# MCG-NJU/MeMOTR

Measured on AMD Instinct MI355X. Metric: train_frames_per_sec, higher is better.
Workload: dtype f32

## Files before the change

### memotr_amd/csrc/clip_ops.hip

```cpp
#include <hip/hip_runtime.h>
#include <stdint.h>
#include <stdio.h>

#include <atomic>

#include "../../include/clip_ops_hip.h"
#include "assign_core.h"

namespace {

thread_local char g_err[256] = {0};

int fail(int code, const char *msg) {
    snprintf(g_err, sizeof(g_err), "%s", msg);
    return code;
}

int check_launch(const char *what) {
    const hipError_t e = hipGetLastError();
    if (e != hipSuccess) {
        snprintf(g_err, sizeof(g_err), "%s: %s", what, hipGetErrorString(e));
        return (int)e;
    }
    g_err[0] = 0;
    return 0;
}

typedef float f32x4_t __attribute__((ext_vector_type(4)));
typedef double f64x4_t __attribute__((ext_vector_type(4)));

struct Box {
    float x1, y1, x2, y2;
};

__device__ __forceinline__ Box to_xyxy(float cx, float cy, float w, float h) {
#pragma clang fp contract(off)
    Box b;
    b.x1 = cx - 0.5f * w;
    b.y1 = cy - 0.5f * h;
    b.x2 = cx + 0.5f * w;
    b.y2 = cy + 0.5f * h;
    return b;
}

__device__ __forceinline__ float giou_pair(const Box a, const Box b) {
#pragma clang fp contract(off)
    const float iw = fmaxf(fminf(a.x2, b.x2) - fmaxf(a.x1, b.x1), 0.f);
    const float ih = fmaxf(fminf(a.y2, b.y2) - fmaxf(a.y1, b.y1), 0.f);
    const float inter = iw * ih;
    const float area_a = (a.x2 - a.x1) * (a.y2 - a.y1);
    const float area_b = (b.x2 - b.x1) * (b.y2 - b.y1);
    const float uni = area_a + area_b - inter;
    const float iou = inter / uni;
    const float hw = fmaxf(fmaxf(a.x2, b.x2) - fminf(a.x1, b.x1), 0.f);
    const float hh = fmaxf(fmaxf(a.y2, b.y2) - fminf(a.y1, b.y1), 0.f);
    const float hull = hw * hh;
    return iou - (hull - uni) / hull;
}

__device__ __forceinline__ float sigmoidf(float x) { return 1.f / (1.f + expf(-x)); }

__device__ __forceinline__ float powg(float x, float gamma) { return gamma == 2.f ? x * x : powf(x, gamma); }

__global__ __launch_bounds__(256) void match_cost_kernel(const float *__restrict__ logits, long lsl, long lsq,
                                                        const float *__restrict__ boxes, long bsl, long bsq,
                                                        const int64_t *__restrict__ gt_labels,
                                                        const float *__restrict__ gt_boxes, int n_layers, int Q,
                                                        int K, int T, float w_class, float w_bbox, float w_giou,
                                                        float *__restrict__ cost) {
#pragma clang fp contract(off)
    const long total = (long)n_layers * Q * T;
    for (long i = (long)blockIdx.x * blockDim.x + threadIdx.x; i < total; i += (long)gridDim.x * blockDim.x) {
        const int t = (int)(i % T);
        const long lq = i / T;
        const int q = (int)(lq % Q), l = (int)(lq / Q);
        long lab = gt_labels[t];
        lab = lab < 0 ? 0 : (lab >= K ? K - 1 : lab);
        const float prob = sigmoidf(logits[l * lsl + q * lsq + lab]);
        const float alpha = 0.25f, gamma = 2.f;
        const float neg = ((1.f - alpha) * powg(prob, gamma)) * (-logf(1.f - prob + 1e-8f));
        const float pos = (alpha * powg(1.f - prob, gamma)) * (-logf(prob + 1e-8f));
        const float c_class = pos - neg;
        const float *pb = boxes + l * bsl + q * bsq;
        const float *tb = gt_boxes + (long)t * 4;
        const float p0 = pb[0], p1 = pb[1], p2 = pb[2], p3 = pb[3];
        const float t0 = tb[0], t1 = tb[1], t2 = tb[2], t3 = tb[3];
        const float c_bbox = ((fabsf(p0 - t0) + fabsf(p1 - t1)) + fabsf(p2 - t2)) + fabsf(p3 - t3);
        const float giou = giou_pair(to_xyxy(p0, p1, p2, p3), to_xyxy(t0, t1, t2, t3));
        cost[i] = (w_bbox * c_bbox + w_class * c_class) + w_giou * (-giou);
    }
}

__global__ __launch_bounds__(256) void pair_box_loss_fwd_kernel(const float *__restrict__ boxes,
                                                               const int64_t *__restrict__ lay,
                                                               const int64_t *__restrict__ qidx, long row_mul,
                                                               long row_add, const float *__restrict__ tgt,
                                                               const int64_t *__restrict__ gidx,
                                                               const float *__restrict__ weight, int n,
                                                               float *__restrict__ l1, float *__restrict__ gl) {
#pragma clang fp contract(off)
    const int i = blockIdx.x * blockDim.x + threadIdx.x;
    if (i >= n) return;
    const float *pb = boxes + (lay[i] * row_mul + row_add + qidx[i]) * 4;
    const float *tb = tgt + (gidx ? gidx[i] : (long)i) * 4;
    const float p0 = pb[0], p1 = pb[1], p2 = pb[2], p3 = pb[3];
    const float t0 = tb[0], t1 = tb[1], t2 = tb[2], t3 = tb[3];
    float a = ((fabsf(p0 - t0) + fabsf(p1 - t1)) + fabsf(p2 - t2)) + fabsf(p3 - t3);
    float g = 1.f - giou_pair(to_xyxy(p0, p1, p2, p3), to_xyxy(t0, t1, t2, t3));
    if (weight) {
        a *= weight[i];
        g *= weight[i];
    }
    l1[i] = a;
    gl[i] = g;
}

__device__ __forceinline__ float iou_pair(const Box a, const Box b) {
#pragma clang fp contract(off)
    const float iw = fmaxf(fminf(a.x2, b.x2) - fmaxf(a.x1, b.x1), 0.f);
    const float ih = fmaxf(fminf(a.y2, b.y2) - fmaxf(a.y1, b.y1), 0.f);
    const float inter = iw * ih;
    const float uni = (a.x2 - a.x1) * (a.y2 - a.y1) + (b.x2 - b.x1) * (b.y2 - b.y1) - inter;
    return inter / uni;
}

__global__ __launch_bounds__(256) void pair_iou_kernel(const float *__restrict__ boxes, const float *__restrict__ tgt,
                                                      const int64_t *__restrict__ gidx, int n,
                                                      float *__restrict__ iou) {
#pragma clang fp contract(off)
    const int i = blockIdx.x * blockDim.x + threadIdx.x;
    if (i >= n) return;
    const float *pb = boxes + (long)i * 4;
    const float *tb = tgt + (gidx ? gidx[i] : (long)i) * 4;
    iou[i] = iou_pair(to_xyxy(pb[0], pb[1], pb[2], pb[3]), to_xyxy(tb[0], tb[1], tb[2], tb[3]));
}

struct HandoverCols {
    int K, C, QW, oB, oR, oO, oM, oS, oQ, oI, W;
};

HandoverCols handover_cols(int K, int C, int use_dab) {
    HandoverCols c;
    c.K = K;
    c.C = C;
    c.QW = use_dab ? C : 2 * C;
    c.oB = K;
    c.oR = K + 4;
    c.oO = K + 8;
    c.oM = c.oO + C;
    c.oS = c.oM + C;
    c.oQ = c.oS + C;
    c.oI = c.oQ + c.QW;
    c.W = c.oI + 1;
    return c;
}

// ... 933 lines not shown
                        lo = sr_bf16(sr_to_bf16(lo)) + sr_bf16((uint16_t)(rw[k] & 0xffffu));
                        hi = sr_bf16(sr_to_bf16(hi)) + sr_bf16((uint16_t)(rw[k] >> 16));
                    }
                    lo = lo < 0.f ? 0.f : lo;
                    hi = hi < 0.f ? 0.f : hi;
                    vw[k] = (unsigned)sr_to_bf16(lo) | ((unsigned)sr_to_bf16(hi) << 16);
                }
                reinterpret_cast<uint4 *>(xp)[i] = v;
            }
        } else {
            for (long i = (long)blockIdx.x * blockDim.x + threadIdx.x; i < HW; i += (long)gridDim.x * blockDim.x) {
                float v = sr_bf16(xp[i]) + b;
                if (RES) v = sr_bf16(sr_to_bf16(v)) + sr_bf16(rp[i]);
                xp[i] = sr_to_bf16(v < 0.f ? 0.f : v);
            }
        }
    }
}


typedef float lb_f32x16 __attribute__((ext_vector_type(16)));

#ifndef MSDA_LB_U
#define MSDA_LB_U 4
#endif
constexpr int LB_U = MSDA_LB_U;

template <bool GX, bool RELU>
__device__ __forceinline__ void linear_bwd_tile(const float *__restrict__ g, const float *__restrict__ y,
                                                const float *__restrict__ Bp, int M, int N, int K, int OUT, int i0, int j0,
                                                float *__restrict__ C, float *__restrict__ gb, float (*s_c)[16][64],
                                                float (*s_b)[32]) {
    const int lane = threadIdx.x & 63, wave = threadIdx.x >> 6;
    const int i = i0 + (lane & 31), j = j0 + (lane & 31), kq = (lane >> 5) * 4;
    const bool iok = i < M, jok = j < N;
    const int chunks = (K + 7) / 8, per = (chunks + 3) / 4;
    const int c_lo = wave * per, c_hi = (c_lo + per) < chunks ? (c_lo + per) : chunks;
    const bool vec = GX && (OUT % 4 == 0);
    lb_f32x16 acc = {0.f, 0.f, 0.f, 0.f, 0.f, 0.f, 0.f, 0.f, 0.f, 0.f, 0.f, 0.f, 0.f, 0.f, 0.f, 0.f};
    float bsum = 0.f;
    for (int c = c_lo; c < c_hi; c += LB_U) {
        float a[LB_U][4], b[LB_U][4], m[LB_U][4];
#pragma unroll
        for (int u = 0; u < LB_U; ++u) {
            const int k0 = (c + u) * 8 + kq;
            const bool cok = c + u < c_hi;
            if (vec) {
                float4 av = {0.f, 0.f, 0.f, 0.f}, mv = {1.f, 1.f, 1.f, 1.f};
                if (cok && iok && k0 < K) {
                    av = *reinterpret_cast<const float4 *>(g + (long)i * OUT + k0);
                    if (RELU) mv = *reinterpret_cast<const float4 *>(y + (long)i * OUT + k0);
                }
                a[u][0] = av.x; a[u][1] = av.y; a[u][2] = av.z; a[u][3] = av.w;
                m[u][0] = mv.x; m[u][1] = mv.y; m[u][2] = mv.z; m[u][3] = mv.w;
            }
#pragma unroll
            for (int q = 0; q < 4; ++q) {
                const int k = k0 + q;
                const bool kok = cok && k < K;
                if (!vec) {
                    const long idx = GX ? (long)i * OUT + k : (long)k * OUT + i;
                    a[u][q] = (iok && kok) ? g[idx] : 0.f;
                    m[u][q] = (RELU && iok && kok) ? y[idx] : 1.f;
                }
                b[u][q] = (jok && kok) ? Bp[(long)k * N + j] : 0.f;
            }
        }
#pragma unroll
        for (int u = 0; u < LB_U; ++u) {
#pragma unroll
            for (int q = 0; q < 4; ++q) {
                const float av = RELU ? (m[u][q] <= 0.f ? 0.f : a[u][q]) : a[u][q];
                acc = __builtin_amdgcn_mfma_f32_32x32x2f32(av, b[u][q], acc, 0, 0, 0);
                bsum += av;
            }
        }
    }
#pragma unroll
    for (int r = 0; r < 16; ++r) s_c[wave][r][lane] = acc[r];
    bsum += __shfl_xor(bsum, 32, 64);
    if (lane < 32) s_b[wave][lane] = bsum;
    __syncthreads();
#pragma unroll
    for (int rr = 0; rr < 4; ++rr) {
        const int r = wave * 4 + rr;
        const float v = (s_c[0][r][lane] + s_c[1][r][lane]) + (s_c[2][r][lane] + s_c[3][r][lane]);
        const int row = i0 + (r & 3) + 8 * (r >> 2) + 4 * (lane >> 5);
        if (row < M && jok) C[(long)row * N + j] = v;
    }
    if (!GX && gb != nullptr && j0 == 0 && wave == 0 && lane < 32 && i0 + lane < M)
        gb[i0 + lane] = (s_b[0][lane] + s_b[1][lane]) + (s_b[2][lane] + s_b[3][lane]);
}

template <bool RELU>
__global__ __launch_bounds__(256) void linear_bwd_kernel(const float *__restrict__ g, const float *__restrict__ y,
                                                         const float *__restrict__ x, const float *__restrict__ w,
                                                         int R, int IN, int OUT, float *__restrict__ gx,
                                                         float *__restrict__ gw, float *__restrict__ gb, int n_gx,
                                                         int gx_tj, int gw_tj) {
    __shared__ float s_c[4][16][64];
    __shared__ float s_b[4][32];
    const int tile = blockIdx.x;
    if (tile < n_gx) {
        linear_bwd_tile<true, RELU>(g, y, w, R, IN, OUT, OUT, (tile / gx_tj) * 32, (tile % gx_tj) * 32, gx, nullptr, s_c, s_b);
    } else {
        const int t = tile - n_gx;
        linear_bwd_tile<false, RELU>(g, y, x, OUT, IN, R, OUT, (t / gw_tj) * 32, (t % gw_tj) * 32, gw, gb, s_c, s_b);
    }
}

template <bool RELU>
__global__ __launch_bounds__(256) void linear_fwd_kernel(const float *__restrict__ x, const float *__restrict__ w,
                                                         const float *__restrict__ bias, int R, int IN, int OUT,
                                                         float *__restrict__ yout, int tj) {
    __shared__ float s_c[4][16][64];
    const int lane = threadIdx.x & 63, wave = threadIdx.x >> 6;
    const int i0 = (blockIdx.x / tj) * 32, j0 = (blockIdx.x % tj) * 32;
    const int i = i0 + (lane & 31), j = j0 + (lane & 31), kq = (lane >> 5) * 4;
    const bool iok = i < R, jok = j < OUT;
    const int chunks = (IN + 7) / 8, per = (chunks + 3) / 4;
    const int c_lo = wave * per, c_hi = (c_lo + per) < chunks ? (c_lo + per) : chunks;
    lb_f32x16 acc = {0.f, 0.f, 0.f, 0.f, 0.f, 0.f, 0.f, 0.f, 0.f, 0.f, 0.f, 0.f, 0.f, 0.f, 0.f, 0.f};
    for (int c = c_lo; c < c_hi; c += LB_U) {
        float4 a[LB_U], b[LB_U];
#pragma unroll
        for (int u = 0; u < LB_U; ++u) {
            const int k0 = (c + u) * 8 + kq;
            const bool kok = c + u < c_hi && k0 < IN;
            a[u] = (iok && kok) ? *reinterpret_cast<const float4 *>(x + (long)i * IN + k0) : float4{0.f, 0.f, 0.f, 0.f};
            b[u] = (jok && kok) ? *reinterpret_cast<const float4 *>(w + (long)j * IN + k0) : float4{0.f, 0.f, 0.f, 0.f};
        }
#pragma unroll
        for (int u = 0; u < LB_U; ++u) {
            acc = __builtin_amdgcn_mfma_f32_32x32x2f32(a[u].x, b[u].x, acc, 0, 0, 0);
            acc = __builtin_amdgcn_mfma_f32_32x32x2f32(a[u].y, b[u].y, acc, 0, 0, 0);
            acc = __builtin_amdgcn_mfma_f32_32x32x2f32(a[u].z, b[u].z, acc, 0, 0, 0);
            acc = __builtin_amdgcn_mfma_f32_32x32x2f32(a[u].w, b[u].w, acc, 0, 0, 0);
        }
    }
#pragma unroll
    for (int r = 0; r < 16; ++r) s_c[wave][r][lane] = acc[r];
    __syncthreads();
    const float bj = (bias != nullptr && jok) ? bias[j] : 0.f;
#pragma unroll
    for (int rr = 0; rr < 4; ++rr) {
        const int r = wave * 4 + rr;
        float v = ((s_c[0][r][lane] + s_c[1][r][lane]) + (s_c[2][r][lane] + s_c[3][r][lane])) + bj;
        if (RELU) v = v < 0.f ? 0.f : v;
        const int row = i0 + (r & 3) + 8 * (r >> 2) + 4 * (lane >> 5);
        if (row < R && jok) yout[(long)row * OUT + j] = v;
    }
}

}

__global__ __launch_bounds__(256) void track_ownership_kernel(const int64_t *__restrict__ tr_ids, int n_tr,
                                                              const int64_t *__restrict__ gt_ids, int n_gt,
                                                              int64_t *__restrict__ matched, float *__restrict__ free_out) {
    for (int i = threadIdx.x; i < n_tr; i += blockDim.x) {
        const int64_t id = tr_ids[i];
        int64_t m = -1;
        for (int j = 0; j < n_gt; ++j)
            if (gt_ids[j] == id) m = j;
        matched[i] = m;
    }
    for (int j = threadIdx.x; j < n_gt; j += blockDim.x) {
        const int64_t id = gt_ids[j];
        bool owned = false;
        for (int i = 0; i < n_tr; ++i) owned = owned || tr_ids[i] == id;
        free_out[j] = owned ? 0.f : 1.f;
    }
}

__global__ __launch_bounds__(256) void focal_labels_kernel(const int64_t *__restrict__ lay, const int64_t *__restrict__ q,
                                                           const int64_t *__restrict__ g, int n_pairs,
                                                           const int64_t *__restrict__ gt_labels, int n_gt,
                                                           const int64_t *__restrict__ matched, int n_tr,
                                                           const unsigned char *__restrict__ late, int n_layers, int nd,
                                                           int K, int64_t *__restrict__ labels) {
    const int nq = nd + n_tr;
    for (int e = threadIdx.x; e < n_layers * nq; e += blockDim.x) {
        const int l = e / nq, c = e - l * nq;
        int64_t v = K;
        if (c >= nd && late[l]) {
            const int64_t m = matched[c - nd];
            if (m >= 0 && m < n_gt) v = gt_labels[m];
        }
        labels[e] = v;
    }
    __syncthreads();
    for (int p = threadIdx.x; p < n_pairs; p += blockDim.x) {
        const int64_t l = lay[p], c = q[p], t = g[p];
        if (l >= 0 && l < n_layers && c >= 0 && c < nq && t >= 0 && t < n_gt) labels[l * nq + c] = gt_labels[t];
    }
}

__global__ __launch_bounds__(256) void result_rows_kernel(const float *__restrict__ boxes, const float *__restrict__ scores,
                                                          const int64_t *__restrict__ ids,
                                                          const int64_t *__restrict__ labels, int n, int K, int64_t frame,
                                                          float ori_w, float ori_h, float score_thresh, float area_thresh,
                                                          float *__restrict__ rows_f, int64_t *__restrict__ rows_i,
                                                          int32_t *__restrict__ counters, int capacity) {
    __shared__ int wave_total[4];
    const int lane = threadIdx.x & 63, wave = threadIdx.x >> 6;
    const int stored0 = counters[0], dropped0 = counters[1];
    int base = 0;
    for (int c0 = 0; c0 < n; c0 += 256) {
        const int i = c0 + (int)threadIdx.x;
        bool keep = false;
        float s = 0.f, cx = 0.f, cy = 0.f, w = 0.f, h = 0.f;
        if (i < n) {
            const float *sc = scores + (long)i * K;
            s = sc[0];
            for (int k = 1; k < K; ++k) {
                const float v = sc[k];
                if (v > s || v != v) s = v;
            }
            cx = boxes[4 * i], cy = boxes[4 * i + 1], w = boxes[4 * i + 2], h = boxes[4 * i + 3];
            const float area = __fmul_rn(__fmul_rn(__fmul_rn(w, ori_w), h), ori_h);
            keep = s > score_thresh && area > area_thresh;
        }
        const unsigned long long m = __ballot(keep);
        const int below = __popcll(m & ((1ull << lane) - 1ull));
        if (lane == 0) wave_total[wave] = __popcll(m);
        __syncthreads();
        int before = 0, total = 0;
        for (int v = 0; v < 4; ++v) {
            const int t = wave_total[v];
            before += v < wave ? t : 0;
            total += t;
        }
        if (keep) {
            const long pos = (long)stored0 + base + before + below;
            if (pos >= 0 && pos < capacity) {
                const float hw = __fmul_rn(0.5f, w), hh = __fmul_rn(0.5f, h);
                float *rf = rows_f + pos * 5;
                rf[0] = __fmul_rn(__fsub_rn(cx, hw), ori_w);
                rf[1] = __fmul_rn(__fsub_rn(cy, hh), ori_h);
                rf[2] = __fmul_rn(__fadd_rn(cx, hw), ori_w);
                rf[3] = __fmul_rn(__fadd_rn(cy, hh), ori_h);
                rf[4] = s;
                int64_t *ri = rows_i + pos * 3;
                ri[0] = frame;
                ri[1] = ids[i];
                ri[2] = labels[i];
            }
        }
        base += total;
        __syncthreads();
    }
    if (threadIdx.x == 0) {
        const int room = stored0 < 0 ? 0 : (capacity > stored0 ? capacity - stored0 : 0);
        const int stored = base < room ? base : room;
        counters[0] = stored0 + stored;
        counters[1] = dropped0 + (base - stored);
    }
}

template <int NW>
__device__ __forceinline__ void bank_ranks(bool flag, int lane, int wave, int *wave_total, int &before, int &total) {
    const unsigned long long m = __ballot(flag);
    const int below = __popcll(m & ((1ull << lane) - 1ull));
    if (lane == 0) wave_total[wave] = __popcll(m);
    __syncthreads();
    before = below;
    total = 0;
    for (int v = 0; v < NW; ++v) {
        const int t = wave_total[v];
        before += v < wave ? t : 0;
        total += t;
    }
}

constexpr int BANK_THREADS = 1024, BANK_WAVES = BANK_THREADS / 64;

__global__ __launch_bounds__(BANK_THREADS) void bank_update_kernel(clipops_bank_model m, clipops_bank bank, int n_det, int cap,
                                                          int K, int C, int use_dab, float det_thresh,
                                                          float track_thresh, int64_t miss_tolerance) {
#pragma clang fp contract(off)
    __shared__ int wave_total[BANK_WAVES], wave_live[BANK_WAVES], pair_row[BANK_THREADS], pair_slot[BANK_THREADS];
    const int b = blockIdx.x, lane = threadIdx.x & 63, wave = threadIdx.x >> 6;
    const int QW = use_dab ? C : 2 * C;
    const long bc = (long)b * cap;
    int64_t *ids = bank.ids + bc, *labels = bank.labels + bc, *dtime = bank.disappear_time + bc;
    int32_t *free_list = bank.free_list + bc;
    float *boxes = bank.boxes + bc * 4, *ref_pts = bank.ref_pts + bc * 4;
    float *logits = bank.logits + bc * K, *scores = bank.scores + bc * K;
    float *out_embed = bank.output_embed + bc * C, *long_mem = bank.long_memory + bc * C;
    float *last_out = bank.last_output + bc * C, *query = bank.query_embed + bc * QW;
    const float *m_logits = m.ptr[CLIPOPS_BK_LOGITS] + b * m.batch_stride[CLIPOPS_BK_LOGITS];
    const float *m_boxes = m.ptr[CLIPOPS_BK_BOXES] + b * m.batch_stride[CLIPOPS_BK_BOXES];
    const float *m_out = m.ptr[CLIPOPS_BK_OUTPUTS] + b * m.batch_stride[CLIPOPS_BK_OUTPUTS];
    const float *m_ref = m.ptr[CLIPOPS_BK_LAST_REF] + b * m.batch_stride[CLIPOPS_BK_LAST_REF];
    const float *m_query = m.ptr[CLIPOPS_BK_QUERIES] + b * m.batch_stride[CLIPOPS_BK_QUERIES];
    const long rs_logits = m.row_stride[CLIPOPS_BK_LOGITS], rs_boxes = m.row_stride[CLIPOPS_BK_BOXES];
    const long rs_out = m.row_stride[CLIPOPS_BK_OUTPUTS], rs_ref = m.row_stride[CLIPOPS_BK_LAST_REF];
    const long rs_query = m.row_stride[CLIPOPS_BK_QUERIES];
    const int64_t next0 = bank.next_id[b];
    const int dropped0 = bank.counters[2 * b + 1];

    int n_free = 0;
    for (int s0 = 0; s0 < cap; s0 += BANK_THREADS) {
        const int s = s0 + (int)threadIdx.x;
        const bool is_free = s < cap && ids[s] < 0;
        int before, total;
        bank_ranks<BANK_WAVES>(is_free, lane, wave, wave_total, before, total);
// ... 490 lines not shown
    const size_t lds = (size_t)2 * L * kPitch * sizeof(float);
    if ((rc = allow_lds(reinterpret_cast<const void *>(mha_fwd_kernel), lds, g_lds_fwd))) return rc;
    hipLaunchKernelGGL(mha_fwd_kernel, dim3((L + kRows - 1) / kRows, H, B), dim3(256), lds, (hipStream_t)stream, q, k, v, q_bs,
                       q_rs, k_bs, k_rs, v_bs, v_rs, key_mask, H, L, scale, out, lse);
    return check_launch("mha_fwd_kernel");
}

int clipops_mha_bwd_f32(const float *q, const float *k, const float *v, long q_bs, long q_rs, long k_bs, long k_rs,
                        long v_bs, long v_rs, const uint8_t *key_mask, const float *out, const float *lse,
                        const float *grad_out, int B, int H, int L, float scale, float *grad_q, long gq_bs, long gq_rs,
                        float *grad_k, long gk_bs, long gk_rs, float *grad_v, long gv_bs, long gv_rs, void *stream) {
    int rc = mha_check(q, k, v, B, H, L);
    if (rc) return rc;
    if ((long)B * L == 0) { g_err[0] = 0; return 0; }
    if (!out || !lse || !grad_out || !grad_q || !grad_k || !grad_v) return fail(1, "clipops_mha_bwd_f32: null pointer");
    const size_t lds_q = (size_t)2 * L * kPitch * sizeof(float);
    const size_t lds_kv = lds_q + (size_t)2 * L * sizeof(float);
    if ((rc = allow_lds(reinterpret_cast<const void *>(mha_bwd_q_kernel), lds_q, g_lds_bq))) return rc;
    if ((rc = allow_lds(reinterpret_cast<const void *>(mha_bwd_kv_kernel), lds_kv, g_lds_bkv))) return rc;
    const dim3 grid((L + kRows - 1) / kRows, H, B);
    hipLaunchKernelGGL(mha_bwd_q_kernel, grid, dim3(256), lds_q, (hipStream_t)stream, q, k, v, q_bs, q_rs, k_bs, k_rs,
                       v_bs, v_rs, key_mask, out, lse, grad_out, H, L, scale, grad_q, gq_bs, gq_rs);
    if ((rc = check_launch("mha_bwd_q_kernel"))) return rc;
    hipLaunchKernelGGL(mha_bwd_kv_kernel, grid, dim3(256), lds_kv, (hipStream_t)stream, q, k, v, q_bs, q_rs, k_bs, k_rs,
                       v_bs, v_rs, key_mask, out, lse, grad_out, H, L, scale, grad_k, gk_bs, gk_rs, grad_v, gv_bs, gv_rs);
    return check_launch("mha_bwd_kv_kernel");
}

int clipops_add_layer_norm_fwd_f32(const float *x, const float *res, const float *gamma, const float *beta, long rows,
                                   float eps, float *sum, float *y, float *stats, void *stream) {
    if (rows < 0) return fail(1, "clipops_add_layer_norm_fwd_f32: negative row count");
    if (rows == 0) { g_err[0] = 0; return 0; }
    if (!x || !res || !gamma || !beta || !sum || !y || !stats) return fail(1, "clipops_add_layer_norm_fwd_f32: null pointer");
    hipLaunchKernelGGL(add_layer_norm_fwd_kernel<false>, dim3((unsigned)((rows + 3) / 4)), dim3(256), 0, (hipStream_t)stream,
                       x, res, gamma, beta, nullptr, rows, eps, sum, y, nullptr, stats);
    return check_launch("add_layer_norm_fwd_kernel");
}

int clipops_add_layer_norm_pos_fwd_f32(const float *x, const float *res, const float *gamma, const float *beta,
                                       const float *pos, long rows, float eps, float *sum, float *y, float *q,
                                       float *stats, void *stream) {
    if (rows < 0) return fail(1, "clipops_add_layer_norm_pos_fwd_f32: negative row count");
    if (rows == 0) { g_err[0] = 0; return 0; }
    if (!x || !res || !gamma || !beta || !pos || !sum || !y || !q || !stats)
        return fail(1, "clipops_add_layer_norm_pos_fwd_f32: null pointer");
    hipLaunchKernelGGL(add_layer_norm_fwd_kernel<true>, dim3((unsigned)((rows + 3) / 4)), dim3(256), 0, (hipStream_t)stream,
                       x, res, gamma, beta, pos, rows, eps, sum, y, q, stats);
    return check_launch("add_layer_norm_fwd_kernel<pos>");
}

int clipops_add_layer_norm_bwd_f32(const float *grad_y, const float *sum, const float *stats, const float *gamma,
                                   long rows, int chunk_rows, float *grad_sum, float *partial, void *stream) {
    if (rows < 0 || chunk_rows <= 0) return fail(1, "clipops_add_layer_norm_bwd_f32: bad dimension");
    if (rows == 0) { g_err[0] = 0; return 0; }
    if (!grad_y || !sum || !stats || !gamma || !grad_sum || !partial)
        return fail(1, "clipops_add_layer_norm_bwd_f32: null pointer");
    hipLaunchKernelGGL(add_layer_norm_bwd_kernel, dim3((unsigned)((rows + chunk_rows - 1) / chunk_rows)), dim3(256), 0,
                       (hipStream_t)stream, grad_y, sum, stats, gamma, rows, chunk_rows, grad_sum, partial);
    return check_launch("add_layer_norm_bwd_kernel");
}

int clipops_add_layer_norm_fanin_bwd_f32(const float *g0, const float *g1, const float *g2, const float *sum,
                                         const float *stats, const float *gamma, long rows, int chunk_rows,
                                         float *grad_sum, float *partial, float *colsum_partial, void *stream) {
    if (rows < 0 || chunk_rows <= 0) return fail(1, "clipops_add_layer_norm_fanin_bwd_f32: bad dimension");
    if (rows == 0) { g_err[0] = 0; return 0; }
    const float *g[3] = {nullptr, nullptr, nullptr};
    int n = 0;
    if (g0) g[n++] = g0;
    if (g1) g[n++] = g1;
    if (g2) g[n++] = g2;
    if (n == 0) return fail(1, "clipops_add_layer_norm_fanin_bwd_f32: no gradient input");
    if (!sum || !stats || !gamma || !grad_sum || !partial || !colsum_partial)
        return fail(1, "clipops_add_layer_norm_fanin_bwd_f32: null pointer");
    hipLaunchKernelGGL(add_layer_norm_bwd_fanin_kernel, dim3((unsigned)((rows + chunk_rows - 1) / chunk_rows)), dim3(256), 0,
                       (hipStream_t)stream, g[0], g[1], g[2], sum, stats, gamma, rows, chunk_rows, grad_sum, partial,
                       colsum_partial);
    return check_launch("add_layer_norm_bwd_fanin_kernel");
}

int clipops_assign_f32(const float *cost, long stride_problem, long stride_row, long stride_col, int n_problems,
                       int n_rows, int n_cols, int32_t *row_ind, int32_t *col_ind, int32_t *status, void *stream) {
    if (n_problems < 0 || n_rows < 0 || n_cols < 0) return fail(1, "clipops_assign_f32: bad dimension");
    if (n_problems == 0 || n_rows == 0 || n_cols == 0) { g_err[0] = 0; return 0; }
    if (!cost || !row_ind || !col_ind) return fail(1, "clipops_assign_f32: null pointer");
    const int nr = n_rows < n_cols ? n_rows : n_cols, nc = n_rows < n_cols ? n_cols : n_rows;
    if (nc > CLIPOPS_ASSIGN_MAX_DIM) return fail(2, "clipops_assign_f32: problem exceeds CLIPOPS_ASSIGN_MAX_DIM");
    const size_t lds = (assign::work_bytes(nr, nc) + 15) & ~(size_t)15;
    if (lds > 64 * 1024) {
        static std::atomic<size_t> allowed{0};
        if (lds > 160 * 1024) return fail(2, "clipops_assign_f32: problem does not fit the LDS of a CU");
        if (lds > allowed.load()) {
            if (hipFuncSetAttribute(reinterpret_cast<const void *>(assign_kernel),
                                    hipFuncAttributeMaxDynamicSharedMemorySize, 160 * 1024) != hipSuccess) {
                (void)hipGetLastError();
                return fail(3, "clipops_assign_f32: hipFuncSetAttribute(MaxDynamicSharedMemorySize) failed");
            }
            allowed.store(160 * 1024);
        }
    }
    hipLaunchKernelGGL(assign_kernel, dim3(n_problems), dim3(64), lds, (hipStream_t)stream, cost, stride_problem,
                       stride_row, stride_col, n_rows, n_cols, row_ind, col_ind, status);
    return check_launch("assign_kernel");
}

static int shift_relu_check(const void *x, const void *shift, long planes, int C, long HW, const char *who) {
    if (planes < 0 || C <= 0 || HW < 0) return fail(1, who);
    if (planes && HW && (!x || !shift)) return fail(1, who);
    return 0;
}

int clipops_shift_relu_f32(float *x, const float *shift, const float *res, long planes, int C, long HW, void *stream) {
    if (shift_relu_check(x, shift, planes, C, HW, "clipops_shift_relu_f32: bad argument")) return 1;
    if (planes == 0 || HW == 0) { g_err[0] = 0; return 0; }
    const int vec = (HW % 4 == 0) && ((uintptr_t)x % 16 == 0) && (!res || (uintptr_t)res % 16 == 0);
    const long per = vec ? HW / 4 : HW;
    const dim3 grid((unsigned)((per + 1023) / 1024 > 64 ? 64 : (per + 1023) / 1024 < 1 ? 1 : (per + 1023) / 1024),
                    (unsigned)(planes > 65535 ? 65535 : planes));
    if (res) hipLaunchKernelGGL(shift_relu_f32_kernel<true>, grid, dim3(256), 0, (hipStream_t)stream, x, shift, res, planes, C, HW, vec);
    else hipLaunchKernelGGL(shift_relu_f32_kernel<false>, grid, dim3(256), 0, (hipStream_t)stream, x, shift, res, planes, C, HW, vec);
    return check_launch("shift_relu_f32_kernel");
}

int clipops_shift_relu_bf16(uint16_t *x, const float *shift, const uint16_t *res, long planes, int C, long HW, void *stream) {
    if (shift_relu_check(x, shift, planes, C, HW, "clipops_shift_relu_bf16: bad argument")) return 1;
    if (planes == 0 || HW == 0) { g_err[0] = 0; return 0; }
    const int vec = (HW % 8 == 0) && ((uintptr_t)x % 16 == 0) && (!res || (uintptr_t)res % 16 == 0);
    const long per = vec ? HW / 8 : HW;
    const dim3 grid((unsigned)((per + 1023) / 1024 > 64 ? 64 : (per + 1023) / 1024 < 1 ? 1 : (per + 1023) / 1024),
                    (unsigned)(planes > 65535 ? 65535 : planes));
    if (res) hipLaunchKernelGGL(shift_relu_bf16_kernel<true>, grid, dim3(256), 0, (hipStream_t)stream, x, shift, res, planes, C, HW, vec);
    else hipLaunchKernelGGL(shift_relu_bf16_kernel<false>, grid, dim3(256), 0, (hipStream_t)stream, x, shift, res, planes, C, HW, vec);
    return check_launch("shift_relu_bf16_kernel");
}

int clipops_linear_bwd_f32(const float *grad_y, const float *y_relu, const float *x, const float *w, int rows,
                           int in_features, int out_features, float *grad_x, float *grad_w, float *grad_b,
                           void *stream) {
    if (rows < 0 || in_features <= 0 || out_features <= 0) return fail(1, "clipops_linear_bwd_f32: bad dimension");
    if (!grad_y || !x || !w) return fail(1, "clipops_linear_bwd_f32: null pointer");
    if (grad_b && !grad_w) return fail(1, "clipops_linear_bwd_f32: grad_b is computed with grad_w");
    const int gx_ti = (rows + 31) / 32, gx_tj = (in_features + 31) / 32;
    const int gw_ti = (out_features + 31) / 32, gw_tj = gx_tj;
    const int n_gx = grad_x ? gx_ti * gx_tj : 0, n_gw = grad_w ? gw_ti * gw_tj : 0;
    if (n_gx + n_gw == 0) { g_err[0] = 0; return 0; }
    if (rows == 0) {
        if (grad_w && hipMemsetAsync(grad_w, 0, sizeof(float) * (size_t)out_features * in_features, (hipStream_t)stream) != hipSuccess)
            return fail(3, "clipops_linear_bwd_f32: memset failed");
        if (grad_b && hipMemsetAsync(grad_b, 0, sizeof(float) * (size_t)out_features, (hipStream_t)stream) != hipSuccess)
            return fail(3, "clipops_linear_bwd_f32: memset failed");
        g_err[0] = 0;
        return 0;
    }
    if (y_relu) hipLaunchKernelGGL(linear_bwd_kernel<true>, dim3(n_gx + n_gw), dim3(256), 0, (hipStream_t)stream, grad_y, y_relu, x, w, rows, in_features, out_features, grad_x, grad_w, grad_b, n_gx, gx_tj, gw_tj);
    else hipLaunchKernelGGL(linear_bwd_kernel<false>, dim3(n_gx + n_gw), dim3(256), 0, (hipStream_t)stream, grad_y, y_relu, x, w, rows, in_features, out_features, grad_x, grad_w, grad_b, n_gx, gx_tj, gw_tj);
    return check_launch("linear_bwd_kernel");
}

int clipops_linear_fwd_f32(const float *x, const float *w, const float *bias, int rows, int in_features,
                           int out_features, int relu, float *y, void *stream) {
    if (rows < 0 || in_features <= 0 || out_features <= 0) return fail(1, "clipops_linear_fwd_f32: bad dimension");
    if (in_features % 4) return fail(2, "clipops_linear_fwd_f32: in_features must be a multiple of 4");
    if (rows == 0) { g_err[0] = 0; return 0; }
    if (!x || !w || !y) return fail(1, "clipops_linear_fwd_f32: null pointer");
    const int ti = (rows + 31) / 32, tj = (out_features + 31) / 32;
    if (relu) hipLaunchKernelGGL(linear_fwd_kernel<true>, dim3(ti * tj), dim3(256), 0, (hipStream_t)stream, x, w, bias, rows, in_features, out_features, y, tj);
    else hipLaunchKernelGGL(linear_fwd_kernel<false>, dim3(ti * tj), dim3(256), 0, (hipStream_t)stream, x, w, bias, rows, in_features, out_features, y, tj);
    return check_launch("linear_fwd_kernel");
}

}
```

### memotr_amd/functions/clip_ops.py

```python
from __future__ import annotations

import ctypes
import os

import torch
import torch.nn.functional as F


def fused(*tensors) -> bool:
    return (os.environ.get("MEMOTR_FUSED_CLIP_OPS", "1") != "0"
            and all(t.is_cuda and (t.dtype == torch.float32 or not t.is_floating_point()) for t in tensors))


def config_key() -> tuple:
    return (os.environ.get("MEMOTR_FUSED_CLIP_OPS", "1"), os.environ.get("MEMOTR_COLSUM_TALL", "1"),
            os.environ.get("MEMOTR_ATTN_KERNELS", "1"), os.environ.get("MEMOTR_FUSED_LN", "1"),
            os.environ.get("MEMOTR_FUSED_SHIFT_RELU", "1"), os.environ.get("MEMOTR_FUSED_LINEAR_BWD", "1"),
            os.environ.get("MEMOTR_FUSED_LINEAR_FWD", "1"))


def _lib():
    from .. import _clip_lib
    return _clip_lib


def _stream(t: torch.Tensor) -> int:
    idx = t.device.index
    if idx is not None and idx != torch.cuda.current_device():
        raise RuntimeError(f"clip_ops: tensor on cuda:{idx} but cuda:{torch.cuda.current_device()} is current; "
                           "call torch.cuda.set_device(tensor.device) (one device per process)")
    return torch.cuda.current_stream(t.device).cuda_stream


def _strides3(t: torch.Tensor):
    if t.dim() != 3 or (t.shape[2] > 1 and t.stride(2) != 1):
        raise RuntimeError("expected a (layers, rows, C) tensor with a dense last axis")
    return t.stride(0), t.stride(1)


def match_cost(logits: torch.Tensor, boxes: torch.Tensor, gt_labels: torch.Tensor, gt_boxes: torch.Tensor,
               w_class: float, w_bbox: float, w_giou: float, out: torch.Tensor = None) -> torch.Tensor:
    n_layers, Q, K = logits.shape
    T = gt_labels.shape[0]
    if out is not None:
        assert out.is_contiguous() and out.dtype == torch.float32 and out.numel() == n_layers * Q * T
        cost = out.view(n_layers, Q, T)
    else:
        cost = torch.empty((n_layers, Q, T), dtype=torch.float32, device=logits.device)
    lsl, lsq = _strides3(logits)
    bsl, bsq = _strides3(boxes)
    gt_labels, gt_boxes = gt_labels.contiguous(), gt_boxes.contiguous()
    L = _lib()
    L.check(L.lib.clipops_match_cost_f32(logits.data_ptr(), lsl, lsq, boxes.data_ptr(), bsl, bsq, gt_labels.data_ptr(),
                                         gt_boxes.data_ptr(), n_layers, Q, K, T, float(w_class), float(w_bbox),
                                         float(w_giou), cost.data_ptr(), _stream(logits)), "clipops_match_cost_f32")
    return cost


def track_ownership(track_ids: torch.Tensor, gt_ids: torch.Tensor, free_out: torch.Tensor = None):
    n_tr, n_gt = track_ids.shape[0], gt_ids.shape[0]
    matched = torch.empty((n_tr,), dtype=torch.int64, device=gt_ids.device)
    free = free_out if free_out is not None else torch.empty((n_gt,), dtype=torch.float32, device=gt_ids.device)
    assert free.is_contiguous() and free.dtype == torch.float32 and free.numel() == n_gt
    track_ids, gt_ids = track_ids.contiguous(), gt_ids.contiguous()
    L = _lib()
    L.check(L.lib.clipops_track_ownership_i64(track_ids.data_ptr(), n_tr, gt_ids.data_ptr(), n_gt, matched.data_ptr(),
                                              free.data_ptr(), _stream(gt_ids)), "clipops_track_ownership_i64")
    return matched, free


def track_ownership_reference(track_ids, gt_ids):
    n_gt = gt_ids.shape[0]
    eq = track_ids[:, None] == gt_ids[None, :]
    order = torch.arange(1, n_gt + 1, device=eq.device)
    return (eq * order).amax(1) - 1 if n_gt > 0 else torch.full_like(track_ids, -1), (~eq.any(0)).to(torch.float32)


def focal_labels(lay: torch.Tensor, q: torch.Tensor, g: torch.Tensor, gt_labels: torch.Tensor, matched_idx,
                 late: torch.Tensor, n_det: int, n_tracks: int, num_classes: int) -> torch.Tensor:
    n_layers = late.shape[0]
    labels = torch.empty((n_layers, n_det + n_tracks), dtype=torch.int64, device=late.device)
    lay, q, g, gt_labels = lay.contiguous(), q.contiguous(), g.contiguous(), gt_labels.contiguous()
    L = _lib()
    L.check(L.lib.clipops_focal_labels_i64(lay.data_ptr(), q.data_ptr(), g.data_ptr(), lay.shape[0], gt_labels.data_ptr(),
                                           gt_labels.shape[0], None if matched_idx is None else matched_idx.contiguous().data_ptr(),
                                           n_tracks, late.contiguous().data_ptr(), n_layers, n_det, num_classes,
                                           labels.data_ptr(), _stream(late)), "clipops_focal_labels_i64")
    return labels


def focal_labels_reference(lay, q, g, gt_labels, matched_idx, late, n_det, n_tracks, num_classes):
    n_layers = late.shape[0]
    labels = torch.full((n_layers, n_det + n_tracks), num_classes, dtype=torch.int64, device=late.device)
    labels[lay, q] = gt_labels[g]
    if n_tracks > 0:
        has = matched_idx >= 0
        tr_lab = torch.where(has, gt_labels[matched_idx.clamp(min=0)] if gt_labels.shape[0] > 0
                             else torch.full_like(matched_idx, num_classes), torch.full_like(matched_idx, num_classes))
        labels[:, n_det:] = torch.where(late[:, None], tr_lab[None, :], labels[:, n_det:])
    return labels


class _PairBoxLoss(torch.autograd.Function):
    @staticmethod
    def forward(ctx, boxes_all, lay, qidx, b, tgt_boxes, gidx, weight):
        n_layers, B, Nq, _ = boxes_all.shape
        n = lay.shape[0]
        l1 = torch.empty((n,), dtype=torch.float32, device=boxes_all.device)
        gl = torch.empty_like(l1)
        L = _lib()
        L.check(L.lib.clipops_pair_box_loss_fwd_f32(
            boxes_all.data_ptr(), lay.data_ptr(), qidx.data_ptr(), B * Nq, b * Nq, tgt_boxes.data_ptr(),
            None if gidx is None else gidx.data_ptr(), None if weight is None else weight.data_ptr(), n,
            l1.data_ptr(), gl.data_ptr(), _stream(boxes_all)), "clipops_pair_box_loss_fwd_f32")
        ctx.save_for_backward(boxes_all, lay, qidx, tgt_boxes, gidx, weight)
        ctx.b = b
        return l1, gl

    @staticmethod
    def backward(ctx, g_l1, g_gl):
        boxes_all, lay, qidx, tgt_boxes, gidx, weight = ctx.saved_tensors
        n_layers, B, Nq, _ = boxes_all.shape
        grad = torch.zeros_like(boxes_all)
        L = _lib()
        L.check(L.lib.clipops_pair_box_loss_bwd_f32(
            boxes_all.data_ptr(), lay.data_ptr(), qidx.data_ptr(), B * Nq, ctx.b * Nq, tgt_boxes.data_ptr(),
            None if gidx is None else gidx.data_ptr(), None if weight is None else weight.data_ptr(), lay.shape[0],
            g_l1.contiguous().data_ptr(), g_gl.contiguous().data_ptr(), grad.data_ptr(), _stream(boxes_all)),
            "clipops_pair_box_loss_bwd_f32")
        return grad, None, None, None, None, None, None


def pair_box_loss(boxes_all: torch.Tensor, lay: torch.Tensor, qidx: torch.Tensor, b: int, tgt_boxes: torch.Tensor,
                  gidx: torch.Tensor = None, weight: torch.Tensor = None):
    if not boxes_all.is_contiguous():
        boxes_all = boxes_all.contiguous()
    return _PairBoxLoss.apply(boxes_all, lay.contiguous(), qidx.contiguous(), int(b), tgt_boxes.contiguous(),
                              None if gidx is None else gidx.contiguous(),
                              None if weight is None else weight.contiguous())


def pair_box_loss_reference(boxes_all, lay, qidx, b, tgt_boxes, gidx=None, weight=None):
    from ..models.criterion import paired_giou
    from ..utils.box_ops import box_cxcywh_to_xyxy
    pb = boxes_all[lay, b, qidx]
    tb = tgt_boxes if gidx is None else tgt_boxes[gidx]
    l1 = F.l1_loss(pb, tb, reduction="none").sum(-1)
    gl = 1 - paired_giou(box_cxcywh_to_xyxy(pb), box_cxcywh_to_xyxy(tb))
    if weight is not None:
        l1, gl = l1 * weight, gl * weight
    return l1, gl


def pair_iou(boxes: torch.Tensor, tgt_boxes: torch.Tensor, gidx: torch.Tensor = None) -> torch.Tensor:
    boxes, tgt_boxes = boxes.detach().contiguous(), tgt_boxes.contiguous()
    n = boxes.shape[0]
    out = torch.empty((n,), dtype=torch.float32, device=boxes.device)
    L = _lib()
    L.check(L.lib.clipops_pair_iou_f32(boxes.data_ptr(), tgt_boxes.data_ptr(), None if gidx is None else
                                       gidx.contiguous().data_ptr(), n, out.data_ptr(), _stream(boxes)),
            "clipops_pair_iou_f32")
    return out


def assign(cost: torch.Tensor):
    if cost.dim() != 3 or cost.dtype != torch.float32 or not cost.is_cuda:
        raise RuntimeError("assign expects a float32 CUDA tensor of shape (problems, rows, cols)")
    P, R, C = cost.shape
    k = min(R, C)
    row = torch.empty((P, k), dtype=torch.int32, device=cost.device)
    col = torch.empty((P, k), dtype=torch.int32, device=cost.device)
# ... 827 lines not shown
```

Baseline: 42.28.

## Stage linear fwd/bwd operand tiles through LDS before MFMA contraction

Adds LDS-staged variants of the fused linear forward and backward MFMA kernels. Each block cooperatively loads A and B K-chunks into shared memory with vectorized float4 loads (ReLU mask applied during staging), then the waves run 32x32x2 MFMA from LDS with double-buffered register reads. This targets the strided and uncoalesced global loads of the direct kernels. The cost is extra dynamic LDS, more barriers and possibly lower occupancy. The path is on by default behind MEMOTR_LINEAR_STAGED, which is also added to the config key.

```diff
diff --git a/memotr_amd/csrc/clip_ops.hip b/memotr_amd/csrc/clip_ops.hip
--- a/memotr_amd/csrc/clip_ops.hip
+++ b/memotr_amd/csrc/clip_ops.hip
@@ -1,7 +1,9 @@
 #include <hip/hip_runtime.h>
 #include <stdint.h>
 #include <stdio.h>
-
+#include <stdlib.h>
+
+#include <algorithm>
 #include <atomic>
 
 #include "../../include/clip_ops_hip.h"
@@ -1241,6 +1243,236 @@
     }
 }
 
+constexpr int LS_S = 16;
+constexpr int LS_RED_FLOATS = 4 * 16 * 64 + 4 * 32;
+
+__host__ __device__ constexpr int ls_pitch(int S) { return 32 * S + 4; }
+__host__ __device__ constexpr int ls_chunks(int K) { return (((K + 7) / 8 + 3) / 4) < LS_S ? (((K + 7) / 8 + 3) / 4) : LS_S; }
+__host__ __device__ constexpr int ls_image(bool row, int S) { return row ? 32 * ls_pitch(S) : 8 * 4 * S * 32; }
+constexpr size_t ls_bytes(bool a_row, bool b_row, int K) {
+    const int n = ls_image(a_row, ls_chunks(K)) + ls_image(b_row, ls_chunks(K));
+    return sizeof(float) * (size_t)(n > LS_RED_FLOATS ? n : LS_RED_FLOATS);
+}
+
+template <bool ROW>
+__device__ __forceinline__ void ls_piece(int w, int it, int b, int S, int per, int K, int lim, int t0, long ld, long &off,
+                                         int &n, int &lds) {
+    const int g8 = threadIdx.x >> 3, f = threadIdx.x & 7;
+    int left;
+    if (ROW) {
+        const int fi = f + 8 * it, t = fi >> 1, cw = b * S + t;
+        const int k0 = 8 * (w * per + cw) + 4 * (fi & 1);
+        left = (fi < 2 * S && cw < per && t0 + g8 < lim) ? K - k0 : 0;
+        off = (long)(t0 + g8) * ld + k0;
+        lds = (fi < 2 * S && cw < per && 8 * (w * per + cw) < K) ? g8 * ls_pitch(S) + 8 * (w * S + t) + 4 * (fi & 1) : -1;
+    } else {
+        const int kr = g8 + 32 * it, cw = b * S + (kr >> 3);
+        const int k = 8 * (w * per + b * S) + kr;
+        left = (kr < 8 * S && cw < per && k < K) ? lim - (t0 + 4 * f) : 0;
+        off = (long)k * ld + t0 + 4 * f;
+        lds = (kr < 8 * S && cw < per && 8 * (w * per + cw) < K) ? (8 * w * S + kr) * 32 + 4 * f : -1;
+    }
+    n = left < 0 ? 0 : (left > 4 ? 4 : left);
+}
+
+template <bool VEC>
+__device__ __forceinline__ float4 ls_load4(const float *__restrict__ src, long off, int n) {
+    float4 v;
+    if (VEC) {
+        v = *reinterpret_cast<const float4 *>(src + (n > 0 ? off : 0));
+        if (n <= 0) v = float4{0.f, 0.f, 0.f, 0.f};
+    } else {
+        v.x = src[n > 0 ? off : 0];
+        v.y = src[n > 1 ? off + 1 : 0];
+        v.z = src[n > 2 ? off + 2 : 0];
+        v.w = src[n > 3 ? off + 3 : 0];
+        v.x = n > 0 ? v.x : 0.f; v.y = n > 1 ? v.y : 0.f; v.z = n > 2 ? v.z : 0.f; v.w = n > 3 ? v.w : 0.f;
+    }
+    return v;
+}
+
+template <bool AROW, bool BROW, bool RELU, bool VEC>
+__device__ __forceinline__ void ls_stage(const float *__restrict__ a_src, const float *__restrict__ y_src, long a_ld,
+                                         int a_lim, int a_t0, const float *__restrict__ b_src, long b_ld, int b_lim,
+                                         int b_t0, int K, int per, int S, int b, float *__restrict__ As,
+                                         float *__restrict__ Bs) {
+    const int n_it = (S + 3) / 4;
+    for (int it0 = 0; it0 < n_it; it0 += 2) {
+        float4 va[2][4], vy[2][4], vb[2][4];
+        int la[2][4], lb[2][4];
+#pragma unroll
+        for (int u = 0; u < 2; ++u) {
+#pragma unroll
+            for (int w = 0; w < 4; ++w) {
+                long off;
+                int n;
+                ls_piece<AROW>(w, it0 + u, b, S, per, K, a_lim, a_t0, a_ld, off, n, la[u][w]);
+                va[u][w] = ls_load4<VEC>(a_src, off, n);
+                if (RELU) vy[u][w] = ls_load4<VEC>(y_src, off, n);
+                ls_piece<BROW>(w, it0 + u, b, S, per, K, b_lim, b_t0, b_ld, off, n, lb[u][w]);
+                vb[u][w] = ls_load4<VEC>(b_src, off, n);
+            }
+        }
+#pragma unroll
+        for (int u = 0; u < 2; ++u) {
+#pragma unroll
+            for (int w = 0; w < 4; ++w) {
+                float4 a = va[u][w];
+                if (RELU) {
+                    const float4 m = vy[u][w];
+                    a.x = m.x <= 0.f ? 0.f : a.x; a.y = m.y <= 0.f ? 0.f : a.y;
+                    a.z = m.z <= 0.f ? 0.f : a.z; a.w = m.w <= 0.f ? 0.f : a.w;
+                }
+                if (la[u][w] >= 0) *reinterpret_cast<float4 *>(As + la[u][w]) = a;
+                if (lb[u][w] >= 0) *reinterpret_cast<float4 *>(Bs + lb[u][w]) = vb[u][w];
+            }
+        }
+    }
+}
+
+template <bool AROW, bool BROW>
+__device__ __forceinline__ void ls_mfma(const float *__restrict__ As, const float *__restrict__ Bs, int S, int n_t,
+                                        lb_f32x16 &acc, float &bsum) {
+    const int lane = threadIdx.x & 63, wave = __builtin_amdgcn_readfirstlane(threadIdx.x >> 6);
+    const int l = lane & 31, kq = (lane >> 5) * 4;
+    n_t = __builtin_amdgcn_readfirstlane(n_t);
+    const float *ap = AROW ? As + l * ls_pitch(S) + 8 * wave * S + kq : As + (8 * wave * S + kq) * 32 + l;
+    const float *bp = BROW ? Bs + l * ls_pitch(S) + 8 * wave * S + kq : Bs + (8 * wave * S + kq) * 32 + l;
+    auto read = [&](int t, float *a, float *b) {
+        if (AROW) {
+            const float4 v = *reinterpret_cast<const float4 *>(ap + 8 * t);
+            a[0] = v.x; a[1] = v.y; a[2] = v.z; a[3] = v.w;
+        } else {
+#pragma unroll
+            for (int q = 0; q < 4; ++q) a[q] = ap[(8 * t + q) * 32];
+        }
+        if (BROW) {
+            const float4 v = *reinterpret_cast<const float4 *>(bp + 8 * t);
+            b[0] = v.x; b[1] = v.y; b[2] = v.z; b[3] = v.w;
+        } else {
+#pragma unroll
+            for (int q = 0; q < 4; ++q) b[q] = bp[(8 * t + q) * 32];
+        }
+    };
+    auto mfma4 = [&](const float *a, const float *b) {
+#pragma unroll
+        for (int q = 0; q < 4; ++q) {
+            acc = __builtin_amdgcn_mfma_f32_32x32x2f32(a[q], b[q], acc, 0, 0, 0);
+            bsum += a[q];
+        }
+    };
+    if (n_t <= 0) return;
+    float a0[4], b0[4], a1[4], b1[4];
+    read(0, a0, b0);
+    int t = 0;
+    for (; t + 2 <= n_t; t += 2) {
+        read(t + 1, a1, b1);
+        mfma4(a0, b0);
+        read(t + 2 < n_t ? t + 2 : t + 1, a0, b0);
+        mfma4(a1, b1);
+    }
+    if (t < n_t) mfma4(a0, b0);
+}
+
+template <bool AROW, bool BROW, bool RELU, bool VEC>
+__device__ __forceinline__ void ls_contract(const float *__restrict__ a_src, const float *__restrict__ y_src, long a_ld,
+                                            int a_lim, int a_t0, const float *__restrict__ b_src, long b_ld, int b_lim,
+                                            int b_t0, int K, float *__restrict__ smem, lb_f32x16 &acc, float &bsum) {
+    const int wave = threadIdx.x >> 6;
+    const int chunks = (K + 7) / 8, per = (chunks + 3) / 4;
+    const int mine = (chunks - wave * per) < per ? (chunks - wave * per) : per;
+    const int S = ls_chunks(K);
+    float *As = smem, *Bs = As + ls_image(AROW, S);
+    for (int b = 0; b * S < per; ++b) {
+        if (b) __syncthreads();
+        ls_stage<AROW, BROW, RELU, VEC>(a_src, y_src, a_ld, a_lim, a_t0, b_src, b_ld, b_lim, b_t0, K, per, S, b, As, Bs);
+        __syncthreads();
+        const int n_t = (mine - b * S) < S ? (mine - b * S) : S;
+        ls_mfma<AROW, BROW>(As, Bs, S, n_t, acc, bsum);
+    }
+    __syncthreads();
+}
+
+template <bool GX, bool RELU, bool VEC>
+__device__ __forceinline__ void linear_bwd_tile_staged(const float *__restrict__ g, const float *__restrict__ y,
+                                                       const float *__restrict__ Bp, int M, int N, int K, int OUT, int i0,
+                                                       int j0, float *__restrict__ C, float *__restrict__ gb,
+                                                       float *__restrict__ smem) {
+    float(*s_c)[16][64] = reinterpret_cast<float(*)[16][64]>(smem);
+    float(*s_b)[32] = reinterpret_cast<float(*)[32]>(smem + 4 * 16 * 64);
+    const int lane = threadIdx.x & 63, wave = threadIdx.x >> 6;
+    const int j = j0 + (lane & 31);
+    const bool jok = j < N;
+    lb_f32x16 acc = {0.f, 0.f, 0.f, 0.f, 0.f, 0.f, 0.f, 0.f, 0.f, 0.f, 0.f, 0.f, 0.f, 0.f, 0.f, 0.f};
+    float bsum = 0.f;
+    ls_contract<GX, false, RELU, VEC>(g, y, OUT, M, i0, Bp, N, N, j0, K, smem, acc, bsum);
+#pragma unroll
+    for (int r = 0; r < 16; ++r) s_c[wave][r][lane] = acc[r];
+    bsum += __shfl_xor(bsum, 32, 64);
+    if (lane < 32) s_b[wave][lane] = bsum;
+    __syncthreads();
+#pragma unroll
+    for (int rr = 0; rr < 4; ++rr) {
+        const int r = wave * 4 + rr;
+        const float v = (s_c[0][r][lane] + s_c[1][r][lane]) + (s_c[2][r][lane] + s_c[3][r][lane]);
+        const int row = i0 + (r & 3) + 8 * (r >> 2) + 4 * (lane >> 5);
+        if (row < M && jok) C[(long)row * N + j] = v;
+    }
+    if (!GX && gb != nullptr && j0 == 0 && wave == 0 && lane < 32 && i0 + lane < M)
+        gb[i0 + lane] = (s_b[0][lane] + s_b[1][lane]) + (s_b[2][lane] + s_b[3][lane]);
+}
+
+template <bool RELU, bool VEC>
+__global__ __launch_bounds__(256) void linear_bwd_staged_kernel(const float *__restrict__ g, const float *__restrict__ y,
+                                                                const float *__restrict__ x, const float *__restrict__ w,
+                                                                int R, int IN, int OUT, float *__restrict__ gx,
+                                                                float *__restrict__ gw, float *__restrict__ gb, int n_gx,
+                                                                int gx_tj, int gw_tj) {
+    extern __shared__ __attribute__((aligned(16))) float s_linear[];
+    const int tile = blockIdx.x;
+    if (tile < n_gx) {
+        linear_bwd_tile_staged<true, RELU, VEC>(g, y, w, R, IN, OUT, OUT, (tile / gx_tj) * 32, (tile % gx_tj) * 32, gx,
+                                                nullptr, s_linear);
+    } else {
+        const int t = tile - n_gx;
+        linear_bwd_tile_staged<false, RELU, VEC>(g, y, x, OUT, IN, R, OUT, (t / gw_tj) * 32, (t % gw_tj) * 32, gw, gb,
+                                                 s_linear);
+    }
+}
+
+template <bool RELU, bool VEC>
+__global__ __launch_bounds__(256) void linear_fwd_staged_kernel(const float *__restrict__ x, const float *__restrict__ w,
+                                                                const float *__restrict__ bias, int R, int IN, int OUT,
+                                                                float *__restrict__ yout, int tj) {
+    extern __shared__ __attribute__((aligned(16))) float s_linear[];
+    float(*s_c)[16][64] = reinterpret_cast<float(*)[16][64]>(s_linear);
+    const int lane = threadIdx.x & 63, wave = threadIdx.x >> 6;
+    const int i0 = (blockIdx.x / tj) * 32, j0 = (blockIdx.x % tj) * 32;
+    const int j = j0 + (lane & 31);
+    const bool jok = j < OUT;
+    lb_f32x16 acc = {0.f, 0.f, 0.f, 0.f, 0.f, 0.f, 0.f, 0.f, 0.f, 0.f, 0.f, 0.f, 0.f, 0.f, 0.f, 0.f};
+    float unused = 0.f;
+    ls_contract<true, true, false, VEC>(x, nullptr, IN, R, i0, w, IN, OUT, j0, IN, s_linear, acc, unused);
+#pragma unroll
+    for (int r = 0; r < 16; ++r) s_c[wave][r][lane] = acc[r];
+    __syncthreads();
+    const float bj = (bias != nullptr && jok) ? bias[j] : 0.f;
+#pragma unroll
+    for (int rr = 0; rr < 4; ++rr) {
+        const int r = wave * 4 + rr;
+        float v = ((s_c[0][r][lane] + s_c[1][r][lane]) + (s_c[2][r][lane] + s_c[3][r][lane])) + bj;
+        if (RELU) v = v < 0.f ? 0.f : v;
+        const int row = i0 + (r & 3) + 8 * (r >> 2) + 4 * (lane >> 5);
+        if (row < R && jok) yout[(long)row * OUT + j] = v;
+    }
+}
+
+bool linear_staged() {
+    const char *e = getenv("MEMOTR_LINEAR_STAGED");
+    return !(e && e[0] == '0' && e[1] == 0);
+}
+
+bool aligned16(const void *p) { return ((uintptr_t)p & 15) == 0; }
 }
 
 __global__ __launch_bounds__(256) void track_ownership_kernel(const int64_t *__restrict__ tr_ids, int n_tr,
@@ -2037,6 +2269,19 @@
         g_err[0] = 0;
         return 0;
     }
+    if (linear_staged()) {
+        static std::atomic<unsigned long long> done[4];
+        const size_t lds = std::max(grad_x ? ls_bytes(true, false, out_features) : 0, grad_w ? ls_bytes(false, false, rows) : 0);
+        const bool vec = in_features % 4 == 0 && out_features % 4 == 0 && aligned16(grad_y) && aligned16(x) &&
+                         aligned16(w) && (!y_relu || aligned16(y_relu));
+        const int which = (y_relu ? 2 : 0) + (vec ? 1 : 0);
+        auto kernel = which == 3 ? linear_bwd_staged_kernel<true, true> : which == 2 ? linear_bwd_staged_kernel<true, false>
+                      : which == 1 ? linear_bwd_staged_kernel<false, true> : linear_bwd_staged_kernel<false, false>;
+        int rc;
+        if ((rc = allow_lds(reinterpret_cast<const void *>(kernel), lds, done[which]))) return rc;
+        hipLaunchKernelGGL(kernel, dim3(n_gx + n_gw), dim3(256), lds, (hipStream_t)stream, grad_y, y_relu, x, w, rows, in_features, out_features, grad_x, grad_w, grad_b, n_gx, gx_tj, gw_tj);
+        return check_launch("linear_bwd_staged_kernel");
+    }
     if (y_relu) hipLaunchKernelGGL(linear_bwd_kernel<true>, dim3(n_gx + n_gw), dim3(256), 0, (hipStream_t)stream, grad_y, y_relu, x, w, rows, in_features, out_features, grad_x, grad_w, grad_b, n_gx, gx_tj, gw_tj);
     else hipLaunchKernelGGL(linear_bwd_kernel<false>, dim3(n_gx + n_gw), dim3(256), 0, (hipStream_t)stream, grad_y, y_relu, x, w, rows, in_features, out_features, grad_x, grad_w, grad_b, n_gx, gx_tj, gw_tj);
     return check_launch("linear_bwd_kernel");
@@ -2049,6 +2294,18 @@
     if (rows == 0) { g_err[0] = 0; return 0; }
     if (!x || !w || !y) return fail(1, "clipops_linear_fwd_f32: null pointer");
     const int ti = (rows + 31) / 32, tj = (out_features + 31) / 32;
+    if (linear_staged()) {
+        static std::atomic<unsigned long long> done[4];
+        const size_t lds = ls_bytes(true, true, in_features);
+        const bool vec = aligned16(x) && aligned16(w);
+        const int which = (relu ? 2 : 0) + (vec ? 1 : 0);
+        auto kernel = which == 3 ? linear_fwd_staged_kernel<true, true> : which == 2 ? linear_fwd_staged_kernel<true, false>
+                      : which == 1 ? linear_fwd_staged_kernel<false, true> : linear_fwd_staged_kernel<false, false>;
+        int rc;
+        if ((rc = allow_lds(reinterpret_cast<const void *>(kernel), lds, done[which]))) return rc;
+        hipLaunchKernelGGL(kernel, dim3(ti * tj), dim3(256), lds, (hipStream_t)stream, x, w, bias, rows, in_features, out_features, y, tj);
+        return check_launch("linear_fwd_staged_kernel");
+    }
     if (relu) hipLaunchKernelGGL(linear_fwd_kernel<true>, dim3(ti * tj), dim3(256), 0, (hipStream_t)stream, x, w, bias, rows, in_features, out_features, y, tj);
     else hipLaunchKernelGGL(linear_fwd_kernel<false>, dim3(ti * tj), dim3(256), 0, (hipStream_t)stream, x, w, bias, rows, in_features, out_features, y, tj);
     return check_launch("linear_fwd_kernel");
diff --git a/memotr_amd/functions/clip_ops.py b/memotr_amd/functions/clip_ops.py
--- a/memotr_amd/functions/clip_ops.py
+++ b/memotr_amd/functions/clip_ops.py
@@ -16,7 +16,7 @@
     return (os.environ.get("MEMOTR_FUSED_CLIP_OPS", "1"), os.environ.get("MEMOTR_COLSUM_TALL", "1"),
             os.environ.get("MEMOTR_ATTN_KERNELS", "1"), os.environ.get("MEMOTR_FUSED_LN", "1"),
             os.environ.get("MEMOTR_FUSED_SHIFT_RELU", "1"), os.environ.get("MEMOTR_FUSED_LINEAR_BWD", "1"),
-            os.environ.get("MEMOTR_FUSED_LINEAR_FWD", "1"))
+            os.environ.get("MEMOTR_FUSED_LINEAR_FWD", "1"), os.environ.get("MEMOTR_LINEAR_STAGED", "1"))
 
 
 def _lib():
```

Result: faster. 43.52, median of 6 (+2.9%).
